# ruc98/Distributed-Data-Parallel-ML-Training

Hardware: AMD Instinct MI355X
Metric: images/sec (whole node) VGG-11 CIFAR-10 (higher is better)
Workload: dtype bf16; 1 GPU; model=vgg11, global_batch=256, per_gpu_batch=256, parallelism=dp1, hipgraph=True, buckets=1, grad_comm=fp32, comm=inline, optimizer=SGD(lr=0.1, momentum=0.9, wd=1e-4) fused

## Files before the change

distributed-data-parallel-ml-training_amd/csrc/bind.cpp:

```cpp
#include <hip/hip_runtime.h>
#include <pybind11/pybind11.h>
#include <pybind11/stl.h>

#include <stdexcept>
#include <string>
#include <tuple>
#include <vector>

#include "runtime/comm.h"

namespace py = pybind11;
using ddp_amd::BucketSpec;
using ddp_amd::RcclComm;
using ddp_amd::Reducer;

#include "kernels/api.h"

template <typename T>
static T* P(uintptr_t v) { return reinterpret_cast<T*>(v); }
static hipStream_t S(uintptr_t v) { return reinterpret_cast<hipStream_t>(v); }
static void check(int rc, const char* what) {
  if (rc != 0) {
    std::string msg = std::string(what) + " failed: ";
    msg += (rc > 0) ? hipGetErrorString((hipError_t)rc) : "invalid arguments";
// ... 469 lines not shown
      return;
    }
    check(ddp_softmax_ce(P<void>(logits), bf16, P<long long>(labels), B, J, P<float>(loss_sum),
                         P<int>(correct), P<void>(dlogits), dlogits_bf16, S(st)), "softmax_ce");
  }, py::arg("logits"), py::arg("bf16"), py::arg("labels"), py::arg("B"), py::arg("J"),
     py::arg("loss_sum"), py::arg("correct"), py::arg("dlogits"), py::arg("dlogits_bf16"),
     py::arg("stream"), py::arg("soft") = py::none());

  m.def("sgd", [](uintptr_t p, uintptr_t g, uintptr_t buf, size_t n, float lr, float momentum,
                  float wd, float grad_scale, int nesterov, uintptr_t st, uintptr_t sched) {
    check(ddp_sgd(P<float>(p), P<float>(g), P<float>(buf), n, lr, momentum, wd, grad_scale,
                  nesterov, P<const ddp_amd::LrSched>(sched), S(st)), "sgd");
  }, py::arg("p"), py::arg("g"), py::arg("buf"), py::arg("n"), py::arg("lr"), py::arg("momentum"),
     py::arg("wd"), py::arg("grad_scale"), py::arg("nesterov"), py::arg("stream"),
     py::arg("sched") = 0);
  m.def("conv_options", [](int stages) { ddp_conv_options(stages); }, py::arg("stages") = 2);
  m.def("conv_tune_set", [](int mode, int M, int N, int K, int tile, int splits, int stages) {
    ddp_conv_tune_set(mode, M, N, K, tile, splits, stages);
  }, py::arg("mode"), py::arg("M"), py::arg("N"), py::arg("K"), py::arg("tile"),
     py::arg("splits"), py::arg("stages") = 0);
  m.def("conv_tune_clear", []() { ddp_conv_tune_clear(); });
  m.def("conv_wgrad_pm_set", [](int on) { ddp_conv_wgrad_pm_set(on); });
  m.def("conv_rows_pm_set", [](int on) { ddp_conv_rows_pm_set(on); });
  m.def("bn_fold_bwd_mb", [](int mb) { ddp_bn_fold_bwd_mb(mb); });
  m.def("bn_fold_grid", [](int blocks) { ddp_bn_fold_grid(blocks); });
  m.def("conv_pair_tune_set", [](int M, int N, int K, int hw, int tile, int sd, int sw) {
    ddp_conv_pair_tune_set(M, N, K, hw, tile, sd, sw);
  });
  m.def("conv_force_tile", [](int t, int stages) { ddp_conv_force_tile(t, stages); },
        py::arg("tile_plus_one"), py::arg("stages") = 0);
#ifdef DDP_CONV_STAMPS
  m.def("conv_stamps_set", [](uintptr_t buf, int cap) { ddp_conv_stamps_set(P<void>(buf), cap); });
#endif
  m.def("pack_conv_weights", [](const std::vector<PackTuple>& descs, uintptr_t st) {
    auto d = pack_descs(descs);
    check(ddp_pack_conv_weights(d.data(), (int)d.size(), S(st)), "pack_conv_weights");
  });
  m.def("sgd_pack", [](uintptr_t items, int n_items, uintptr_t descs, uintptr_t p, uintptr_t g,
                       uintptr_t buf, float lr, float momentum, float wd, float grad_scale,
                       int nesterov, uintptr_t st, int zero_grad, uintptr_t counter, int delta,
                       uintptr_t skip, uintptr_t shadow, uintptr_t slot, uintptr_t done,
                       uintptr_t signal, uintptr_t sched, int sched_advance, uintptr_t lars_side,
                       uintptr_t lars_tensors, uintptr_t lars_partial, uintptr_t lars_trust,
                       float lars_eta, float lars_eps, uintptr_t clip_partial, int clip_chunks,
                       float clip_max_norm, float clip_eps, int clip_flags,
                       uintptr_t clip_stats, uintptr_t ema, float ema_one_minus_decay) {
// ... 247 lines not shown
```

distributed-data-parallel-ml-training_amd/csrc/kernels/api.h:

```cpp
#pragma once
#include <hip/hip_runtime.h>
#include <stddef.h>
#include <stdint.h>

namespace ddp_amd {

#ifdef DDP_AMD_DETERMINISTIC
constexpr int kStatRep = 4096;
constexpr bool kDeterministic = true;
#else
constexpr int kStatRep = 16;
constexpr bool kDeterministic = false;
#endif

struct ConvGeom {
  int N, H, W, C;
  int K;
  int R, S, stride, pad;
  int P, Q;
  int Creal;
  int wkrsc;
};

struct BnArgs {
// ... 277 lines not shown
void ddp_conv_epi_stage_set(int on);
int ddp_bn_pool3_fwd(const ddp_amd::BnArgs* a, unsigned char* idx, hipStream_t st);
int ddp_bn_pool3_bwd(const ddp_amd::BnArgs* a, const unsigned char* idx, hipStream_t st);
void ddp_conv_pair_mode(int mode, int items);
void ddp_sgd_fuse_register(float* dw, const ddp_amd::SgdFuse* f, int clear);
void ddp_sgd_fuse_begin();
int ddp_l0_ok(const ddp_amd::ConvGeom* g);
int ddp_l0_fwd(const ddp_amd::ConvGeom* g, const ddp_amd::L0Io* io, hipStream_t st);
int ddp_l0_bwd(const ddp_amd::ConvGeom* g, const ddp_amd::L0Io* io, hipStream_t st);
int ddp_conv_wgrad_final(const ddp_amd::ConvGeom* g, const void* dy, const void* x, float* dw,
                         float* ws, size_t ws_elems, int splits, hipStream_t st);
int ddp_sgd_fuse_taken(uintptr_t* out, int cap);
int ddp_sgd_fuse_take_final(const float* dw, ddp_amd::SgdFuse* out);
int ddp_sgd_fuse_taken_master(uintptr_t* out, int cap);
void ddp_conv_pair_force(int splits_dg, int splits_wg, int tile);
int ddp_conv_bwd_pair(const ddp_amd::ConvGeom* g, const void* dy, const void* wc, void* dx,
                      const void* x, float* dw, float* ws, size_t ws_elems,
                      const ddp_amd::BnBwdFuse* bn, const ddp_amd::BnBwdApply* ba, int* bn_done,
                      hipStream_t st);
void ddp_conv_tune_set(int mode, int M, int N, int K, int tile, int splits, int stages);
void ddp_conv_pair_tune_set(int M, int N, int K, int hw, int tile, int sd, int sw);
void ddp_conv_wgrad_pm_set(int on);
void ddp_conv_rows_pm_set(int on);
void ddp_bn_fold_bwd_mb(int mb);
void ddp_bn_fold_grid(int blocks);
int ddp_conv_dense2x2_ok(const ddp_amd::ConvGeom* g);
void ddp_conv_dense2x2_set(int on);
void ddp_conv_tune_clear();
void ddp_conv_force_tile(int tile_plus_one, int stages);
#ifdef DDP_CONV_STAMPS
void ddp_conv_stamps_set(void* buf, int cap);
#endif
int ddp_pack_conv_weights(const ddp_amd::PackDesc* descs, int n, hipStream_t st);
int ddp_sgd_pack(const ddp_amd::UpdateLaunch* u, hipStream_t st);
int ddp_grad_sumsq(const void* items, int n_items, const float* g, float grad_scale,
                   float* partial, hipStream_t st);
int ddp_lars_norms(const void* items, int n_items, const float* p, const float* g,
                   float grad_scale, void* partial, hipStream_t st);
int ddp_shard_tail(const void* segs, int n_segs, const float* src, float* dst,
                   const ddp_amd::PackDesc* pack, int n_pack, unsigned* done, unsigned* signal,
                   const unsigned* skip, hipStream_t st);
void ddp_sgd_tile_dims(int RS, int* TK, int* TC);
int ddp_sgd_tile_limit();
int ddp_counter_add(int* c, int delta, ddp_amd::LrSched* sched, int sched_mode, hipStream_t st);
int ddp_synth_generate(unsigned char* images, int* labels, int n, int pix_per_img,
                       unsigned int seed, int classes, hipStream_t st);
// ... 25 lines not shown
```

distributed-data-parallel-ml-training_amd/csrc/kernels/common.h:

```cpp
#pragma once
#include <hip/hip_runtime.h>
#include <stdint.h>
#include <cstdlib>

#include "api.h"

namespace ddp_amd {

typedef __bf16 bf16x8 __attribute__((ext_vector_type(8)));
typedef float f32x4 __attribute__((ext_vector_type(4)));
typedef float f32x16 __attribute__((ext_vector_type(16)));
typedef unsigned short u16x8 __attribute__((ext_vector_type(8)));

constexpr int kWave = 64;

#ifdef DDP_AMD_DEBUG
#define DDP_DEVICE_CHECK(cond)                                                              \
  do {                                                                                      \
    if (!(cond)) {                                                                          \
      printf("[ddp_amd debug] %s:%d check failed: %s (block %d thread %d)\n", __FILE__,     \
             __LINE__, #cond, (int)blockIdx.x, (int)threadIdx.x);                           \
      return;                                                                               \
    }                                                                                       \
  } while (0)
#else
#define DDP_DEVICE_CHECK(cond) \
  do {                        \
  } while (0)
// ... 60 lines not shown
}
__device__ __forceinline__ float dpp_sum16(float v) {
  v += dpp_f<0xB1>(v);
  v += dpp_f<0x4E>(v);
  v += dpp_f<0x141>(v);
  v += dpp_f<0x140>(v);
  return v;
}
__device__ __forceinline__ float lane_f(float v, int l) {
  return __int_as_float(__builtin_amdgcn_readlane(__float_as_int(v), l));
}
__device__ __forceinline__ float wave_sum(float v) {
  v = dpp_sum16(v);
  return (lane_f(v, 0) + lane_f(v, 16)) + (lane_f(v, 32) + lane_f(v, 48));
}
__device__ __forceinline__ float wave_max(float v) {
  v = fmaxf(v, dpp_f<0xB1>(v));
  v = fmaxf(v, dpp_f<0x4E>(v));
  v = fmaxf(v, dpp_f<0x141>(v));
  v = fmaxf(v, dpp_f<0x140>(v));
  return fmaxf(fmaxf(lane_f(v, 0), lane_f(v, 16)), fmaxf(lane_f(v, 32), lane_f(v, 48)));
}

__device__ __forceinline__ int xcd_remap(int orig, int nwg) {
  const int nx = 8;
  if (nwg < nx) return orig;
  const int q = nwg / nx, r = nwg % nx;
  const int xcd = orig % nx, idx = orig / nx;
  return (xcd < r ? xcd * (q + 1) : r * (q + 1) + (xcd - r) * q) + idx;
}

struct FastDiv {
  unsigned mul;
  int sh;
};
__device__ __forceinline__ int fast_div(int x, FastDiv d) {
  return (int)((__umulhi((unsigned)x, d.mul) + (unsigned)x) >> d.sh);
}
inline FastDiv make_fastdiv(int d) {
  FastDiv f;
  int sh = 0;
  while ((1ll << sh) < d) ++sh;
  f.sh = sh;
  f.mul = (unsigned)((((1ull << sh) - (unsigned long long)d) << 32) / (unsigned long long)d + 1);
  return f;
}

#ifdef DDP_CONV_STAMPS
struct ConvStampBuf {
  unsigned* buf;
  int cap;
};
extern ConvStampBuf g_conv_stamps;
__device__ __forceinline__ unsigned long long stamp_now() {
  __builtin_amdgcn_sched_barrier(0);
  const unsigned long long t = __builtin_readcyclecounter();
  __builtin_amdgcn_sched_barrier(0);
  return t;
}
__device__ __forceinline__ void stamp_put(const ConvStampBuf& s, unsigned tag, unsigned long long t0,
                                          unsigned long long t1, unsigned long long t2,
                                          unsigned long long t3) {
  if (!s.buf || threadIdx.x != 0) return;
  const unsigned i = atomicAdd(s.buf, 1u);
  if (i >= (unsigned)s.cap) return;
  unsigned* r = s.buf + 4 + 4 * (size_t)i;
  r[0] = tag;
  r[1] = (unsigned)(t1 - t0);
  r[2] = (unsigned)(t2 - t1);
  r[3] = (unsigned)(t3 - t2);
// ... 15 lines not shown
```

distributed-data-parallel-ml-training_amd/csrc/kernels/conv_igemm.hip:

```cpp
#include "common.h"
#include "api.h"
#include "linear_blocks.h"
#include <algorithm>
#include <map>
#include <set>
#include <cstdlib>

namespace ddp_amd {

enum { MODE_FWD = 0, MODE_DGRAD = 1, MODE_WGRAD = 2 };

typedef short v4i16 __attribute__((ext_vector_type(4)));
typedef short short8_t __attribute__((ext_vector_type(8)));
typedef __attribute__((address_space(3))) v4i16 lds_v4i16;

__global__ __launch_bounds__(256) void zero16_kernel(uint4* __restrict__ p, size_t n16) {
  for (size_t i = blockIdx.x * 256ull + threadIdx.x; i < n16; i += (size_t)gridDim.x * 256)
    p[i] = (uint4){0u, 0u, 0u, 0u};
}

__device__ __forceinline__ void ld8f_conv(const float* p, float* v) {
  const float4 a = reinterpret_cast<const float4*>(p)[0];
  const float4 b = reinterpret_cast<const float4*>(p)[1];
  v[0] = a.x; v[1] = a.y; v[2] = a.z; v[3] = a.w;
  v[4] = b.x; v[5] = b.y; v[6] = b.z; v[7] = b.w;
}
// ... 10 lines not shown
  int Mg, Ng, Kg;
  int splits;
  int ksteps_per_split;
  int phase;
  int pa, pb, Hp, Wp, r0, s0, Rt, St, qa, qb;
  int accumulate;
  int a_bytes, b_bytes;
  FastDiv dPQ, dQ;
  int has_bnf;
  BnBwdFuse bnf;
  const BnFwdFuse* bnfwd;
  int* bnfwd_done;
  const BnBwdApply* bnapply;
  int* bnapply_done;
  int epi_stage;
  int d2x2;
  int d2C, d2K;
  int no_finish;
  const unsigned short* acc_dy;
  const unsigned char* acc_mask;
  SgdFuse sgd;
  int pixmajor;
  FastDiv dTiles, dTilesN, dN, dCdim, dKb, dSdec, dS, dC, dNb, dD2C, dD2K, dSplits;
  int w_dq, w_dp;
#ifdef DDP_CONV_STAMPS
  ConvStampBuf stamps;
#endif
};

__device__ __forceinline__ uint2 acc_old4(const unsigned short* dx, const unsigned short* acc_dy,
                                          const unsigned char* acc_mask, size_t e) {
  if (!acc_mask) return *reinterpret_cast<const uint2*>(dx + e);
  uint2 v = *reinterpret_cast<const uint2*>(acc_dy + e);
  const unsigned mb = (unsigned)acc_mask[e >> 3] >> (e & 4);
  v.x &= ((mb & 1u) ? 0xFFFFu : 0u) | ((mb & 2u) ? 0xFFFF0000u : 0u);
  v.y &= ((mb & 4u) ? 0xFFFFu : 0u) | ((mb & 8u) ? 0xFFFF0000u : 0u);
  return v;
}
__device__ __forceinline__ u16x8 acc_old8(const unsigned short* dx, const unsigned short* acc_dy,
                                          const unsigned char* acc_mask, size_t e) {
  if (!acc_mask) return ld8(dx + e);
  u16x8 v = ld8(acc_dy + e);
  const unsigned mb = acc_mask[e >> 3];
#pragma unroll
  for (int i = 0; i < 8; ++i) v[i] = ((mb >> i) & 1u) ? v[i] : (unsigned short)0;
  return v;
// ... 72 lines not shown

__device__ __forceinline__ void dma_buf(__amdgpu_buffer_rsrc_t rs, int byte_off,
                                        unsigned short* lds_wave_base) {
  __builtin_amdgcn_raw_ptr_buffer_load_lds(rs, (lds_void*)lds_wave_base, 16, byte_off, 0, 0, 0);
}
__device__ __forceinline__ void dma_buf_s(__amdgpu_buffer_rsrc_t rs, int byte_off, int soff,
                                          unsigned short* lds_wave_base) {
  __builtin_amdgcn_raw_ptr_buffer_load_lds(rs, (lds_void*)lds_wave_base, 16, byte_off,
                                           __builtin_amdgcn_readfirstlane(soff), 0, 0);
}

template <int N>
__device__ __forceinline__ void wait_dma_barrier() {
  asm volatile("s_waitcnt vmcnt(%0)\n\ts_barrier" ::"n"(N) : "memory");
}

template <int BM, int BN, int NST>
struct ConvSmem {
  static constexpr int elems = NST * (BM + BN) * 64;
};

template <int MODE, int BM, int BN, int NST, int BNF = 0, bool XSTAT = false, bool SGDM = false>
__device__ __forceinline__ void conv_igemm_body(const ConvArgs& args, unsigned short* smem,
                                                const int bid, const int nblk) {
  constexpr int BK = 64;
  constexpr int WTM = BM / 2, WTN = BN / 2;
  constexpr bool kOldBnf = BNF == 1 || (BNF == 2 && BM == 64 && BN == 64);
  constexpr int TM = WTM / 16, TN = WTN / 16;
  constexpr int CA = BM * BK / 8 / 256;
  constexpr int CB = BN * BK / 8 / 256;
  constexpr int TILE_A = BM * BK, TILE_B = BN * BK;
  constexpr int STAGE = TILE_A + TILE_B;
  static_assert(CA >= 1 && CB >= 1, "tile too small for 256 threads");
  static_assert(NST >= 2 && NST <= 4, "2..4 LDS stages");

  const int tid = threadIdx.x;
  const int lane = tid & 63;
  const int wid = __builtin_amdgcn_readfirstlane(tid >> 6);
  const int wm = wid >> 1, wn = wid & 1;
  DDP_DEVICE_CHECK(blockDim.x == 256 && args.g.C % 8 == 0 && args.g.K % 8 == 0);
  DDP_DEVICE_CHECK(args.splits >= 1 && args.ksteps_per_split >= 1);

  const int tiles_n = (args.Ng + BN - 1) / BN;
  const int tiles_m = (args.Mg + BM - 1) / BM;
  const int tiles = tiles_m * tiles_n;
  const int nitems = tiles * args.splits;
  const int ksteps = (args.Kg + BK - 1) / BK;

  f32x4 acc[TM][TN];
  const ConvGeom& gg = args.g;

  constexpr int NA = (MODE != MODE_WGRAD) ? CA : 1;
  int a_off[CA];
  int a_h0[NA], a_w0[NA];
  int b_off[CB];
  int kr = 0, ks_ = 0, kc = 0;
  KInfo xk;
  int xk_same = 0;
  int wp[CB], wq[CB];
  int w_rr = 0, w_ss = 0, w_lim = 0;
  const bool wsame = MODE == MODE_WGRAD && gg.stride == 1 && gg.P == gg.H && gg.Q == gg.W;
  const int w_dq = args.w_dq;
  const int w_dp = args.w_dp;
  const int w_dm = wsame ? 2 * BK * gg.C : 0;
  const bool pm = MODE == MODE_WGRAD && args.pixmajor;
  const bool pmr = MODE != MODE_WGRAD && args.pixmajor;
  int pmr_pq = 0, pmr_n0 = 0, pmr_row0 = 0, pmr_t = 0;
  int pmr_pp = 0, pmr_qq = 0;
  unsigned pmr_mask = 0;
  int pm_p = 0, pm_q = 0, pm_qlo = 0, pm_qhi = 0, pm_n0 = 0, pm_r = 0, pm_s = 0;
  int row0 = 0, col0 = 0, zsplit = 0, ks_begin = 0, ks_end = 0, cur_tile = 0;
  int d2pos = 0;
  const bool phase = MODE == MODE_DGRAD && args.phase;
  const int Sdec = phase ? args.St : gg.S;
  const int cdim = MODE == MODE_FWD ? gg.C : gg.K;
  const bool fast = MODE != MODE_WGRAD && (cdim % BK) == 0;
  const int lcA = (MODE != MODE_WGRAD) ? ((tid & 7) ^ ((tid >> 4) & 7))
                                       : ((tid % (BM / 8)) ^ mc_swz<BM>(tid / (BM / 8)));
  constexpr bool BKM = MODE != MODE_FWD;
  const int lcB = !BKM ? lcA : ((tid % (BN / 8)) ^ mc_swz<BN>(tid / (BN / 8)));
  const __amdgpu_buffer_rsrc_t rsA = make_rsrc(args.a, args.a_bytes);
  const __amdgpu_buffer_rsrc_t rsB = make_rsrc(args.b, args.b_bytes);

  auto setup = [&](int item) {
    zsplit = fast_div(item, args.dTiles);
    const int tile = xcd_remap(item - zsplit * tiles, tiles);
    cur_tile = tile;
    const int tm = fast_div(tile, args.dTilesN);
    const int tn = tile - tm * tiles_n;
    row0 = tm * BM;
    col0 = tn * BN;
    ks_begin = zsplit * args.ksteps_per_split;
    ks_end = min(ksteps, ks_begin + args.ksteps_per_split);
    if (MODE != MODE_WGRAD) {
      if (pmr) {
        pmr_pq = fast_div(row0, args.dN);
        pmr_n0 = row0 - pmr_pq * gg.N;
        pmr_row0 = row0;
        pmr_pp = fast_div(pmr_pq, args.dQ);
        pmr_qq = pmr_pq - pmr_pp * gg.Q;
        const int img = MODE == MODE_FWD ? gg.H * gg.W * gg.C : gg.P * gg.Q * gg.K;
#pragma unroll
        for (int i = 0; i < CA; ++i) a_off[i] = 2 * (((tid >> 3) + 32 * i) * img + lcA * 8);
      } else {
#pragma unroll
        for (int i = 0; i < CA; ++i) {
          const RowInfo ri = row_info<MODE>(args, row0 + (tid >> 3) + 32 * i);
          a_h0[i] = ri.h0;
          a_w0[i] = ri.w0;
          const int e = (MODE == MODE_FWD) ? ri.base + (ri.h0 * gg.W + ri.w0) * gg.C
                                           : ri.base + (ri.h0 * gg.Q + ri.w0) * gg.K;
          a_off[i] = 2 * (e + (fast ? lcA * 8 : 0));
// ... 716 lines not shown
    }
  }
  if (red) {
    __syncthreads();
    if (wm == 0 && rl == 0) {
      float* st = (MODE == MODE_FWD ? args.stats : args.bnf.sums) +
                  stat_rep(bid) * 2 * args.Ng;
#pragma unroll
      for (int j = 0; j < TN; ++j) {
        const int col = col0 + wn * WTN + j * 16 + cq;
        if (col >= args.Ng) continue;
        const float* slot = reinterpret_cast<const float*>(smem) + (((wn * TN + j) * 4 + (lane >> 4)) * 8);
#pragma unroll
        for (int t = 0; t < 4; ++t) {
          atomicAdd(st + col + t, stat_val(stat_s[j][t] + slot[t], bid));
          atomicAdd(st + args.Ng + col + t, stat_val(stat_ss[j][t] + slot[4 + t], bid));
        }
      }
    }
  }
  };

  constexpr int DMA = CA + CB;
  for (int item = bid; item < nitems; item += nblk) {
#ifdef DDP_CONV_STAMPS
    const unsigned long long st0 = stamp_now();
#endif
    setup(item);
#ifdef DDP_CONV_STAMPS
    const unsigned long long st1 = stamp_now();
#endif
#pragma unroll
    for (int i = 0; i < TM; ++i)
#pragma unroll
      for (int j = 0; j < TN; ++j) acc[i][j] = (f32x4){0.f, 0.f, 0.f, 0.f};
    const int kb = ks_begin, ke = ks_end;
#pragma unroll
    for (int s = 0; s < NST - 1; ++s)
      if (kb + s < ke) issue(kb + s, s);
    int stage = 0;
    for (int ks = kb; ks < ke; ++ks) {
      const int ahead = ke - 1 - ks;
      if (NST >= 4 && ahead >= 2) wait_dma_barrier<(NST >= 4 ? 2 : 0) * DMA>();
      else if (NST >= 3 && ahead >= 1) wait_dma_barrier<(NST >= 3 ? 1 : 0) * DMA>();
      else wait_dma_barrier<0>();
      bf16x8 fa0[TM], fb0[TN], fa1[TM], fb1[TN];
      load_frags(stage, 0, fa0, fb0);
      if (ks + NST - 1 < ke) issue(ks + NST - 1, stage == 0 ? NST - 1 : stage - 1);
      load_frags(stage, 32, fa1, fb1);
      mma(fa0, fb0);
      mma(fa1, fb1);
// ... 19 lines not shown
#define DDP_CONV_WAVES_PER_EU 2
#endif
template <int MODE, int BM, int BN, int NST, int BNF = 0, bool XSTAT = false>
__global__ __launch_bounds__(256) __attribute__((amdgpu_waves_per_eu(DDP_CONV_WAVES_PER_EU)))
void conv_igemm_kernel(ConvArgs args) {
  extern __shared__ __attribute__((aligned(16))) unsigned short smem[];
  conv_igemm_body<MODE, BM, BN, NST, BNF, XSTAT>(args, smem, blockIdx.x, gridDim.x);
}

template <int MODE, int BM, int BN, int NST>
__global__ __launch_bounds__(256) __attribute__((amdgpu_waves_per_eu(2)))
void conv_igemm_bnf2_kernel(ConvArgs args) {
  extern __shared__ __attribute__((aligned(16))) unsigned short smem[];
  conv_igemm_body<MODE, BM, BN, NST, 2>(args, smem, blockIdx.x, gridDim.x);
}

template <int BM, int BN, int NST, int BNF, bool SGDM = false>
__global__ __launch_bounds__(256) void conv_bwd_pair_kernel(ConvArgs dg, ConvArgs wg, int n_dg) {
  __shared__ __attribute__((aligned(16))) unsigned short smem[ConvSmem<BM, BN, NST>::elems];
  if ((int)blockIdx.x < n_dg)
    conv_igemm_body<MODE_DGRAD, BM, BN, NST, BNF>(dg, smem, blockIdx.x, n_dg);
  else
    conv_igemm_body<MODE_WGRAD, BM, BN, NST, 0, false, SGDM>(wg, smem, blockIdx.x - n_dg,
                                                           gridDim.x - n_dg);
}
struct RowMap {
  int stride, Hp, Wp, H, W, pa, pb;
};

__device__ __forceinline__ size_t map_row(const RowMap& m, int row) {
  if (m.stride == 0) return row;
  const int hw = m.Hp * m.Wp;
  const int n = row / hw, rem = row - n * hw;
  const int i = rem / m.Wp, j = rem - i * m.Wp;
  return ((size_t)n * m.H + m.pa + m.stride * i) * m.W + m.pb + m.stride * j;
}

constexpr int kSlabBatch = 8;
__device__ __forceinline__ void sum_slabs8(const float* p, size_t slab, int z0, int z1, float* v) {
  for (int zb = z0; zb < z1; zb += kSlabBatch) {
    float4 a[kSlabBatch], b[kSlabBatch];
#pragma unroll
    for (int u = 0; u < kSlabBatch; ++u) {
      if (zb + u < z1) {
        const float4* src = reinterpret_cast<const float4*>(p + (size_t)(zb + u) * slab);
        a[u] = src[0];
        b[u] = src[1];
// ... 662 lines not shown
  const double eff = (BM == 128 && BN == 128) ? 1.0 : ((BM == 64 && BN == 64) ? 0.55 : 0.8);
  const int resident = (BM == 128 && BN == 128) ? 2 : ((BM == 64 && BN == 64) ? 4 : 3);
  const double blocks = (double)tiles * splits;
  const double fill = std::min(1.0, blocks / (256.0 * resident));
  const double work = (double)tiles * BM * BN * ksteps * 64.0;
  const double t_mfma = work / (eff * fill) / 1.0e15 * 2.0;
  double t_split = 0.0;
  if (splits > 1) t_split = 8.0 * splits * (double)slab / 4.0e12 + 3.0e-6;
  return t_mfma + t_split;
}

static int stages_for(int BM, int BN) {
  if (g_stages <= 2) return 2;
  if (BM == 128 && BN == 128) return g_stages >= 4 ? 4 : 2;
  if (BM == 64 && BN == 64) return g_stages >= 4 ? 4 : 3;
  return 3;
}

static int fwd_stat_grid() {
  constexpr int g = 2048;
  return (kDeterministic ? std::min(g, kStatRep) : g) / 8 * 8;
}

template <int MODE, int BM, int BN, int NST, int BNF>
static void launch_gemm_t(const ConvArgs& a, int items, hipStream_t st) {
  constexpr int kStageBytes = (BM + BN) * 64 * 2;
  constexpr int kTileBytes = BM * BN * 2;
  const int stages = std::max(1, std::min(NST, a.ksteps_per_split));
  size_t lds = (size_t)stages * kStageBytes;
  if (a.epi_stage && lds < (size_t)kTileBytes) lds = kTileBytes;
  int grid = items;
  if (MODE == MODE_FWD && a.stats && a.splits <= 1 && a.epi_stage && !(BM == 64 && BN == 64) &&
      fwd_stat_grid() > 0 && items > fwd_stat_grid())
    grid = fwd_stat_grid();
  void (*kern)(ConvArgs);
  if constexpr (BNF == 2 && MODE == MODE_DGRAD) kern = conv_igemm_bnf2_kernel<MODE, BM, BN, NST>;
  else if constexpr (MODE == MODE_FWD && BNF == 0 && !(BM == 64 && BN == 64))
    kern = grid < items ? conv_igemm_kernel<MODE, BM, BN, NST, 0, true>
                        : conv_igemm_kernel<MODE, BM, BN, NST, 0, false>;
  else kern = conv_igemm_kernel<MODE, BM, BN, NST, BNF>;
  static bool attr[2] = {false, false};
  if (!attr[grid < items]) {
    (void)hipFuncSetAttribute(reinterpret_cast<const void*>(kern),
                              hipFuncAttributeMaxDynamicSharedMemorySize,
                              std::max(NST * kStageBytes, kTileBytes));
    attr[grid < items] = true;
  }
  hipLaunchKernelGGL(kern, dim3(grid), dim3(256), lds, st, a);
}

template <int MODE, int BM, int BN, int NST>
static void launch_gemm(const ConvArgs& a, int items, hipStream_t st) {
  if constexpr (MODE == MODE_DGRAD) {
    if (a.has_bnf && a.splits <= 1)
      return a.bnf.pool ? launch_gemm_t<MODE, BM, BN, NST, 1>(a, items, st)
                        : launch_gemm_t<MODE, BM, BN, NST, 2>(a, items, st);
  }
// ... 42 lines not shown
  {
    const ConvGeom& g = a.g;
    const int cdim = MODE == MODE_FWD ? g.C : g.K;
    const bool wsame = MODE == MODE_WGRAD && g.stride == 1 && g.P == g.H && g.Q == g.W;
    a.dTiles = make_fastdiv(std::max(1, tiles));
    a.dTilesN = make_fastdiv(std::max(1, (a.Ng + BN - 1) / BN));
    a.dN = make_fastdiv(std::max(1, g.N));
    a.dCdim = make_fastdiv(std::max(1, cdim));
    a.dKb = make_fastdiv(std::max(1, cdim / BK));
    a.dSdec = make_fastdiv(std::max(1, MODE == MODE_DGRAD && a.phase ? a.St : g.S));
    a.dS = make_fastdiv(std::max(1, g.S));
    a.dC = make_fastdiv(std::max(1, g.C));
    a.dNb = make_fastdiv(std::max(1, g.N / BK));
    a.dD2C = make_fastdiv(std::max(1, a.d2C));
    a.dD2K = make_fastdiv(std::max(1, a.d2K));
    a.dSplits = make_fastdiv(splits);
    a.w_dq = wsame ? BK % g.Q : 0;
    a.w_dp = wsame ? (BK / g.Q) % g.P : 0;
  }
#ifdef DDP_CONV_STAMPS
  a.stamps = g_conv_stamps;
#endif
  return tiles * splits;
}

static bool needs_finish(int mode, const ConvArgs& a) {
  (void)mode;
  return a.splits > 1;
}

static int finish_rows_per_thread(int Mg, int rows_per_block) {
  return (Mg + rows_per_block - 1) / rows_per_block <= 128 ? 1 : 2;
}

static void dg_finish_grid(const ConvArgs& a, int* bx_out, int* chunks_out) {
  const int G = a.Ng / 8;
  const int Gb = G < 256 ? G : 256;
  const int chunks = (G + Gb - 1) / Gb;
  const int rows_per_block = std::max(1, 256 / Gb);
  const int rpt = finish_rows_per_thread(a.Mg, rows_per_block);
  int bx = (a.Mg + rows_per_block * rpt - 1) / (rows_per_block * rpt);
  *bx_out = std::max(1, std::min(bx, 2048 / chunks + 1));
  *chunks_out = chunks;
}

static FinishArgs finish_args(int mode, const ConvArgs& a) {
// ... 119 lines not shown
    hipLaunchKernelGGL(wgrad_finish_krsc_kernel, dim3(w.gx, w.gy), dim3(256), 0, st, a.ws,
                       a.splits, a.g.K, a.g.R * a.g.S, a.g.C, a.g.Creal, a.dw, w.sgd);
  } else if (MODE == MODE_WGRAD) {
    const int groups = (a.splits + kWgFinishGroup - 1) / kWgFinishGroup;
    const size_t lds = sizeof(float) * a.g.R * a.g.S * a.g.C;
    hipLaunchKernelGGL(wgrad_finish_kernel, dim3(a.g.K, groups), dim3(256), lds, st, a.ws,
                       a.splits, a.g.K, a.g.R, a.g.S, a.g.C, a.g.Creal, a.dw);
  } else {
    if (MODE == MODE_FWD && a.bnfwd && launch_finish_bnfwd(a, st)) return;
    if (MODE == MODE_DGRAD && a.has_bnf && a.bnapply && launch_finish_bnbwd(a, st, nullptr)) return;
    int bx, chunks;
    dg_finish_grid(a, &bx, &chunks);
    const FinishArgs fa = finish_args(MODE, a);
    if (MODE == MODE_DGRAD && a.has_bnf)
      hipLaunchKernelGGL(splitk_finish_kernel<true>, dim3(bx, chunks), dim3(256), 0, st, fa);
    else
      hipLaunchKernelGGL(splitk_finish_kernel<false>, dim3(bx, chunks), dim3(256), 0, st, fa);
  }
}

template <int MODE, int BM, int BN>
static void launch_cfg(ConvArgs& a, int splits, hipStream_t st, int nst_req = 0) {
  const int items = prepare_cfg<MODE, BM, BN>(a, splits);
  constexpr int kStageBytes = (BM + BN) * 64 * 2;
  constexpr int kMaxStages = kStageBytes * 4 <= 163840 ? 4 : (kStageBytes * 3 <= 163840 ? 3 : 2);
  int nst = nst_req >= 2 && nst_req <= 4 ? nst_req : stages_for(BM, BN);
  nst = std::min(nst, kMaxStages);
  if constexpr (kMaxStages >= 4) {
    if (nst == 4) { launch_gemm<MODE, BM, BN, 4>(a, items, st); goto launched; }
  }
  if constexpr (kMaxStages >= 3) {
    if (nst == 3) { launch_gemm<MODE, BM, BN, 3>(a, items, st); goto launched; }
  }
  launch_gemm<MODE, BM, BN, 2>(a, items, st);
launched:
  if (!a.no_finish) launch_finish<MODE>(a, st);
}

struct TuneKey {
  int mode, M, N, K;
  int hw = 0;
  bool operator<(const TuneKey& o) const {
    if (mode != o.mode) return mode < o.mode;
    if (M != o.M) return M < o.M;
    if (N != o.N) return N < o.N;
    if (K != o.K) return K < o.K;
// ... 423 lines not shown
}

constexpr int kPairTiles = 6;
template <int BM, int BN, int NST, bool BNF1, bool SGDM>
static void pair_kernel_launch(const ConvArgs& d, const ConvArgs& w, int itd, int itw,
                               hipStream_t st) {
  hipLaunchKernelGGL((conv_bwd_pair_kernel<BM, BN, NST, BNF1 ? 1 : 0, SGDM>), dim3(itd + itw),
                     dim3(256), 0, st, d, w, itd);
}
template <int BM, int BN, int NST>
static void pair_launch_t(ConvArgs& d, ConvArgs& w, int sd, int sw, float* ws, size_t ws_elems,
                          int* itd_out, int* itw_out, bool* ok_out, const float* dw,
                          bool launch, hipStream_t st) {
  const int itd = prepare_cfg<MODE_DGRAD, BM, BN>(d, std::max(1, sd));
  size_t dneed = needs_finish(MODE_DGRAD, d) ? (size_t)d.splits * d.Mg * d.Ng : 0;
  dneed = (dneed + 63) / 64 * 64;
  w.ws = ws + dneed;
  const int itw = prepare_cfg<MODE_WGRAD, BM, BN>(w, std::max(1, sw));
  const size_t wneed = needs_finish(MODE_WGRAD, w) ? (size_t)w.splits * w.Mg * w.Ng : 0;
  *itd_out = itd;
  *itw_out = itw;
  *ok_out = dneed + wneed <= ws_elems;
  if (!launch || !*ok_out) return;
  if (!needs_finish(MODE_WGRAD, w) && w.g.wkrsc && w.g.Creal == w.g.C) w.sgd = sgd_fuse_master(dw);
  const bool bnf1 = d.has_bnf && d.splits <= 1;
  const bool sgdm = w.sgd.p != nullptr;
  if (bnf1 && sgdm) pair_kernel_launch<BM, BN, NST, true, true>(d, w, itd, itw, st);
  else if (bnf1) pair_kernel_launch<BM, BN, NST, true, false>(d, w, itd, itw, st);
  else if (sgdm) pair_kernel_launch<BM, BN, NST, false, true>(d, w, itd, itw, st);
  else pair_kernel_launch<BM, BN, NST, false, false>(d, w, itd, itw, st);
}

extern "C" int ddp_conv_bwd_pair(const ConvGeom* g, const void* dy, const void* wc, void* dx,
                                 const void* x, float* dw, float* ws, size_t ws_elems,
                                 const BnBwdFuse* bn, const BnBwdApply* ba, int* bn_done,
                                 hipStream_t st) {
  if (bn_done) *bn_done = 0;
  if (!bn) ba = nullptr;
  auto separate = [&]() -> int {
    const BnBwdFuse* bsep = bn && bn->code ? nullptr : bn;
    const int r = conv_dgrad_impl(g, dy, wc, dx, ws, ws_elems, 0, 0, bsep, bsep ? ba : nullptr,
                                  bn_done, st);
    if (r) return r;
    g_sgd_allow = true;
    const int rw = ddp_conv_wgrad(g, dy, x, dw, ws, ws_elems, 0, st);
    g_sgd_allow = false;
// ... 165 lines not shown
```

distributed-data-parallel-ml-training_amd/csrc/kernels/conv_tr.hip:

```cpp
#include "common.h"
#include "api.h"

#include <algorithm>
#include <cstdlib>
#include <map>
#include <tuple>

namespace ddp_amd {
namespace tr {

typedef __attribute__((address_space(3))) void lds_void;

constexpr unsigned kOOB = 0x80000000u;

__device__ __forceinline__ __amdgpu_buffer_rsrc_t make_rsrc(const void* base, int bytes) {
  return __builtin_amdgcn_make_buffer_rsrc(const_cast<void*>(base), (short)0, bytes, 0x00020000);
}

__device__ __forceinline__ void dma(__amdgpu_buffer_rsrc_t rs, unsigned byte_off, unsigned short* lds) {
  __builtin_amdgcn_raw_ptr_buffer_load_lds(rs, (lds_void*)lds, 16, (int)byte_off, 0, 0, 0);
}

template <int N>
__device__ __forceinline__ void wait_dma_barrier() {
// ... 24 lines not shown
  int N, H, W, C, K;
  const unsigned short* x;
  const unsigned short* wc;
  const float* bias;
  unsigned short* z;
  float* stats;
  float* ws;
  int splits, cbps;
  int imgs, rows, bands;
  int imgp, plane, zslot;
  int x_bytes, w_bytes;
  int tiles_m, tiles_n;
  int abuf_elems;
  const unsigned short* zin;
  const float* in_stats;
  const float* in_gamma;
  const float* in_beta;
  float in_eps;
  int in_relu;
  float* in_coef;
  unsigned short* y_out;
  int z_bytes;
  FastDiv dTiles, dTilesN, dBands, dPw, dW, dPerImg;
#ifdef DDP_CONV_STAMPS
  ConvStampBuf stamps;
#endif
};

template <int BM, int BN, int NST, int NL, int IN>
#ifndef DDP_TR_WAVES_PER_EU
#define DDP_TR_WAVES_PER_EU 1
#endif
__global__ __launch_bounds__(256) __attribute__((amdgpu_waves_per_eu(DDP_TR_WAVES_PER_EU)))
void conv_tr_fwd_kernel(Args a) {
  constexpr int WTM = BM / 2, WTN = BN / 2, TM = WTM / 16, TN = WTN / 16;
  constexpr int CB = BN * 64 / 8 / 256;
  constexpr int BTILE = BN * 64;
  static_assert(CB >= 1 && TM >= 1 && TN >= 1, "tile");
  static_assert(NST >= 3 && NST <= 9, "the next patch is issued at tap 0: at most one in the window");
  extern __shared__ __attribute__((aligned(16))) unsigned short smem[];
  const int aelems = a.abuf_elems;
  unsigned short* abuf = smem;
  unsigned short* bring = smem + 2 * aelems;
  float* cf = reinterpret_cast<float*>(bring + NST * BTILE);
  constexpr int NP = IN == 2 ? 4 : 1;
  constexpr bool BNIN = IN == 1 || IN == 2;

  const int tid = threadIdx.x, lane = tid & 63;
  const int wid = __builtin_amdgcn_readfirstlane(tid >> 6);
  const int wm = wid >> 1, wn = wid & 1;
  const int W = a.W, H = a.H, C = a.C, K = a.K;
  const int M = a.N * H * W;
#ifdef DDP_CONV_STAMPS
  const unsigned long long st0 = stamp_now();
#endif
  const int ncb = C / 64;

  const int tiles = a.tiles_m * a.tiles_n;
  const int item = blockIdx.x;
  const int sp = fast_div(item, a.dTiles);
  const int tile = xcd_remap(item - sp * tiles, tiles);
  const int tm = fast_div(tile, a.dTilesN);
  const int tn = tile - tm * a.tiles_n;
  const int row0 = tm * BM, col0 = tn * BN;
  const int cb0 = sp * a.cbps, cb1 = min(ncb, cb0 + a.cbps);
  const int nsteps = (cb1 - cb0) * 9;
  const int tband = fast_div(tm, a.dBands);
  const int n0 = tband * a.imgs;
  const int h0 = (tm - tband * a.bands) * a.rows;

  const __amdgpu_buffer_rsrc_t rsA = IN ? make_rsrc(a.zin, a.z_bytes) : make_rsrc(a.x, a.x_bytes);
  if (BNIN) {
    const int Hz = IN == 2 ? 2 * H : H, Wz = IN == 2 ? 2 * W : W;
    const float Mz = (float)a.N * Hz * Wz;
    for (int c = tid; c < C; c += 256) {
      float s1 = 0.f, s2 = 0.f;
#pragma unroll
      for (int r = 0; r < kStatRep; ++r) {
        s1 += a.in_stats[r * 2 * C + c];
        s2 += a.in_stats[r * 2 * C + C + c];
      }
      const float mu = s1 / Mz;
      const float var = fmaxf(s2 / Mz - mu * mu, 0.f);
      const float is = rsqrtf(var + a.in_eps);
      const float sc = a.in_gamma[c] * is, sh = a.in_beta[c] - mu * sc;
      cf[c] = sc;
// ... 511 lines not shown
  Args a{};
  a.N = N; a.H = H; a.W = W; a.C = C; a.K = K;
  a.x = (const unsigned short*)x;
  a.wc = (const unsigned short*)wc;
  a.bias = bias;
  a.z = (unsigned short*)z;
  a.stats = stats;
  a.ws = ws;
  a.splits = pl.splits;
  a.cbps = pl.cbps;
  a.imgs = geo.imgs; a.rows = geo.rows; a.bands = geo.bands;
  a.imgp = geo.imgp; a.plane = geo.plane; a.zslot = geo.zslot;
  a.x_bytes = (int)(2 * M * C);
  a.w_bytes = (int)(2 * (size_t)K * 9 * C);
  a.abuf_elems = geo.abuf;
  a.tiles_m = (int)(M / c.bm);
  a.tiles_n = K / c.bn;
  a.dTiles = make_fastdiv(std::max(1, a.tiles_m * a.tiles_n));
  a.dTilesN = make_fastdiv(std::max(1, a.tiles_n));
  a.dBands = make_fastdiv(std::max(1, geo.bands));
  a.dPw = make_fastdiv((geo.rows + 2) * W);
  a.dW = make_fastdiv(W);
  a.dPerImg = make_fastdiv(geo.rows * W);
  if (in) {
    a.zin = (const unsigned short*)in->z;
    a.in_stats = in->stats;
    a.in_gamma = in->gamma;
    a.in_beta = in->beta;
    a.in_eps = in->eps;
    a.in_relu = in->relu;
    a.in_coef = in->coef;
    a.y_out = (unsigned short*)in->y;
    a.z_bytes = (int)(2 * M * C * (in->pool ? 4 : 1));
  }
#ifdef DDP_CONV_STAMPS
  a.stamps = g_conv_stamps;
#endif
  const int items = a.tiles_m * a.tiles_n * pl.splits;
  if (!launch_stages(c, in_mode, a, geo.nl, items, st)) return 0;
  int e = (int)hipGetLastError();
  if (e) return 2 + e;
  if (pl.splits > 1) {
    e = ddp_conv_fwd_finish(g, ws, pl.splits, bias, z, stats, bn, bn_done, st);
    if (e) return 2 + e;
  }
  return 1;
// ... 16 lines not shown
```

Baseline: 380,500 images/s.

## Choose conv work-item ordering per XCD via host-side L2 traffic model

```diff
diff --git a/distributed-data-parallel-ml-training_amd/csrc/bind.cpp b/distributed-data-parallel-ml-training_amd/csrc/bind.cpp
--- a/distributed-data-parallel-ml-training_amd/csrc/bind.cpp
+++ b/distributed-data-parallel-ml-training_amd/csrc/bind.cpp
@@ -515,6 +515,7 @@
   m.def("conv_tune_clear", []() { ddp_conv_tune_clear(); });
   m.def("conv_wgrad_pm_set", [](int on) { ddp_conv_wgrad_pm_set(on); });
   m.def("conv_rows_pm_set", [](int on) { ddp_conv_rows_pm_set(on); });
+  m.def("conv_item_order", [](int order) { ddp_conv_item_order(order); });
   m.def("bn_fold_bwd_mb", [](int mb) { ddp_bn_fold_bwd_mb(mb); });
   m.def("bn_fold_grid", [](int blocks) { ddp_bn_fold_grid(blocks); });
   m.def("conv_pair_tune_set", [](int M, int N, int K, int hw, int tile, int sd, int sw) {
diff --git a/distributed-data-parallel-ml-training_amd/csrc/kernels/api.h b/distributed-data-parallel-ml-training_amd/csrc/kernels/api.h
--- a/distributed-data-parallel-ml-training_amd/csrc/kernels/api.h
+++ b/distributed-data-parallel-ml-training_amd/csrc/kernels/api.h
@@ -323,6 +323,8 @@
 void ddp_conv_pair_tune_set(int M, int N, int K, int hw, int tile, int sd, int sw);
 void ddp_conv_wgrad_pm_set(int on);
 void ddp_conv_rows_pm_set(int on);
+void ddp_conv_item_order(int order);
+int ddp_conv_item_order_get();
 void ddp_bn_fold_bwd_mb(int mb);
 void ddp_bn_fold_grid(int blocks);
 int ddp_conv_dense2x2_ok(const ddp_amd::ConvGeom* g);
diff --git a/distributed-data-parallel-ml-training_amd/csrc/kernels/common.h b/distributed-data-parallel-ml-training_amd/csrc/kernels/common.h
--- a/distributed-data-parallel-ml-training_amd/csrc/kernels/common.h
+++ b/distributed-data-parallel-ml-training_amd/csrc/kernels/common.h
@@ -4,6 +4,7 @@
 #include <cstdlib>
 
 #include "api.h"
+#include "conv_item_map.h"
 
 namespace ddp_amd {
 
@@ -110,30 +111,6 @@
   return fmaxf(fmaxf(lane_f(v, 0), lane_f(v, 16)), fmaxf(lane_f(v, 32), lane_f(v, 48)));
 }
 
-__device__ __forceinline__ int xcd_remap(int orig, int nwg) {
-  const int nx = 8;
-  if (nwg < nx) return orig;
-  const int q = nwg / nx, r = nwg % nx;
-  const int xcd = orig % nx, idx = orig / nx;
-  return (xcd < r ? xcd * (q + 1) : r * (q + 1) + (xcd - r) * q) + idx;
-}
-
-struct FastDiv {
-  unsigned mul;
-  int sh;
-};
-__device__ __forceinline__ int fast_div(int x, FastDiv d) {
-  return (int)((__umulhi((unsigned)x, d.mul) + (unsigned)x) >> d.sh);
-}
-inline FastDiv make_fastdiv(int d) {
-  FastDiv f;
-  int sh = 0;
-  while ((1ll << sh) < d) ++sh;
-  f.sh = sh;
-  f.mul = (unsigned)((((1ull << sh) - (unsigned long long)d) << 32) / (unsigned long long)d + 1);
-  return f;
-}
-
 #ifdef DDP_CONV_STAMPS
 struct ConvStampBuf {
   unsigned* buf;
diff --git a/distributed-data-parallel-ml-training_amd/csrc/kernels/conv_igemm.hip b/distributed-data-parallel-ml-training_amd/csrc/kernels/conv_igemm.hip
--- a/distributed-data-parallel-ml-training_amd/csrc/kernels/conv_igemm.hip
+++ b/distributed-data-parallel-ml-training_amd/csrc/kernels/conv_igemm.hip
@@ -2,6 +2,7 @@
 #include "api.h"
 #include "linear_blocks.h"
 #include <algorithm>
+#include <array>
 #include <map>
 #include <set>
 #include <cstdlib>
@@ -58,6 +59,7 @@
   SgdFuse sgd;
   int pixmajor;
   FastDiv dTiles, dTilesN, dN, dCdim, dKb, dSdec, dS, dC, dNb, dD2C, dD2K, dSplits;
+  int item_order;
   int w_dq, w_dp;
 #ifdef DDP_CONV_STAMPS
   ConvStampBuf stamps;
@@ -176,7 +178,8 @@
 
 template <int MODE, int BM, int BN, int NST, int BNF = 0, bool XSTAT = false, bool SGDM = false>
 __device__ __forceinline__ void conv_igemm_body(const ConvArgs& args, unsigned short* smem,
-                                                const int bid, const int nblk) {
+                                                const int bid, const int nblk,
+                                                const int first = 0) {
   constexpr int BK = 64;
   constexpr int WTM = BM / 2, WTN = BN / 2;
   constexpr bool kOldBnf = BNF == 1 || (BNF == 2 && BM == 64 && BN == 64);
@@ -200,7 +203,6 @@
   const int tiles = tiles_m * tiles_n;
   const int nitems = tiles * args.splits;
   const int ksteps = (args.Kg + BK - 1) / BK;
-
   f32x4 acc[TM][TN];
   const ConvGeom& gg = args.g;
 
@@ -236,12 +238,14 @@
   const __amdgpu_buffer_rsrc_t rsA = make_rsrc(args.a, args.a_bytes);
   const __amdgpu_buffer_rsrc_t rsB = make_rsrc(args.b, args.b_bytes);
 
-  auto setup = [&](int item) {
-    zsplit = fast_div(item, args.dTiles);
-    const int tile = xcd_remap(item - zsplit * tiles, tiles);
-    cur_tile = tile;
-    const int tm = fast_div(tile, args.dTilesN);
-    const int tn = tile - tm * tiles_n;
+  auto setup = [&](int k) {
+    const int order = args.item_order;
+    const item_map::Walk walk = item_map::walk_begin(order, first + bid, first, nblk, nitems);
+    const item_map::Dims dims{tiles_m, tiles_n, args.splits, args.dTiles, args.dTilesN};
+    const int lin = walk.base + k * walk.stride;
+    int tm, tn;
+    item_map::decode(order, lin, dims, &zsplit, &tm, &tn);
+    cur_tile = tm * tiles_n + tn;
     row0 = tm * BM;
     col0 = tn * BN;
     ks_begin = zsplit * args.ksteps_per_split;
@@ -1004,11 +1008,11 @@
   };
 
   constexpr int DMA = CA + CB;
-  for (int item = bid; item < nitems; item += nblk) {
+  for (int item = bid, k = 0; item < nitems; item += nblk, ++k) {
 #ifdef DDP_CONV_STAMPS
     const unsigned long long st0 = stamp_now();
 #endif
-    setup(item);
+    setup(k);
 #ifdef DDP_CONV_STAMPS
     const unsigned long long st1 = stamp_now();
 #endif
@@ -1074,7 +1078,7 @@
     conv_igemm_body<MODE_DGRAD, BM, BN, NST, BNF>(dg, smem, blockIdx.x, n_dg);
   else
     conv_igemm_body<MODE_WGRAD, BM, BN, NST, 0, false, SGDM>(wg, smem, blockIdx.x - n_dg,
-                                                           gridDim.x - n_dg);
+                                                           gridDim.x - n_dg, n_dg);
 }
 struct RowMap {
   int stride, Hp, Wp, H, W, pa, pb;
@@ -1783,6 +1787,14 @@
   return (kDeterministic ? std::min(g, kStatRep) : g) / 8 * 8;
 }
 
+template <int MODE, int BM, int BN>
+static int gemm_grid(const ConvArgs& a, int items) {
+  if (MODE == MODE_FWD && a.stats && a.splits <= 1 && a.epi_stage && !(BM == 64 && BN == 64) &&
+      fwd_stat_grid() > 0 && items > fwd_stat_grid())
+    return fwd_stat_grid();
+  return items;
+}
+
 template <int MODE, int BM, int BN, int NST, int BNF>
 static void launch_gemm_t(const ConvArgs& a, int items, hipStream_t st) {
   constexpr int kStageBytes = (BM + BN) * 64 * 2;
@@ -1790,10 +1802,7 @@
   const int stages = std::max(1, std::min(NST, a.ksteps_per_split));
   size_t lds = (size_t)stages * kStageBytes;
   if (a.epi_stage && lds < (size_t)kTileBytes) lds = kTileBytes;
-  int grid = items;
-  if (MODE == MODE_FWD && a.stats && a.splits <= 1 && a.epi_stage && !(BM == 64 && BN == 64) &&
-      fwd_stat_grid() > 0 && items > fwd_stat_grid())
-    grid = fwd_stat_grid();
+  const int grid = gemm_grid<MODE, BM, BN>(a, items);
   void (*kern)(ConvArgs);
   if constexpr (BNF == 2 && MODE == MODE_DGRAD) kern = conv_igemm_bnf2_kernel<MODE, BM, BN, NST>;
   else if constexpr (MODE == MODE_FWD && BNF == 0 && !(BM == 64 && BN == 64))
@@ -1882,6 +1891,36 @@
   a.stamps = g_conv_stamps;
 #endif
   return tiles * splits;
+}
+
+static int g_item_order = -1;
+extern "C" void ddp_conv_item_order(int order) {
+  g_item_order = order >= 0 && order < item_map::kNumOrders ? order : -1;
+}
+extern "C" int ddp_conv_item_order_get() { return g_item_order; }
+template <int MODE, int BM, int BN>
+static void choose_item_order(ConvArgs& a, int first, int nblk) {
+  const ConvGeom& g = a.g;
+  item_map::ModelProblem p{};
+  p.mode = MODE;
+  p.N = g.N; p.H = g.H; p.W = g.W; p.C = g.C; p.K = g.K; p.R = g.R; p.S = g.S; p.pad = g.pad;
+  p.Mg = a.Mg; p.Ng = a.Ng; p.Kg = a.Kg;
+  p.BM = BM; p.BN = BN;
+  p.splits = a.splits;
+  p.ksteps_per_split = a.ksteps_per_split;
+  p.pixmajor = a.pixmajor;
+  p.first = first;
+  p.nblk = nblk;
+  int order = g_item_order;
+  if (order < 0 || !item_map::order_ok(p, order)) {
+    static std::map<std::array<int, 18>, int> cache;
+    const std::array<int, 18> key{MODE, g.N, g.H, g.W, g.C, g.K, g.R * 64 + g.S, g.pad, a.Mg, a.Ng,
+                                  a.Kg, BM, BN, a.splits, a.ksteps_per_split, a.pixmajor, first, nblk};
+    auto it = cache.find(key);
+    if (it == cache.end()) it = cache.emplace(key, item_map::model_choose(p)).first;
+    order = it->second;
+  }
+  a.item_order = order;
 }
 
 static bool needs_finish(int mode, const ConvArgs& a) {
@@ -2047,6 +2086,7 @@
 template <int MODE, int BM, int BN>
 static void launch_cfg(ConvArgs& a, int splits, hipStream_t st, int nst_req = 0) {
   const int items = prepare_cfg<MODE, BM, BN>(a, splits);
+  choose_item_order<MODE, BM, BN>(a, 0, gemm_grid<MODE, BM, BN>(a, items));
   constexpr int kStageBytes = (BM + BN) * 64 * 2;
   constexpr int kMaxStages = kStageBytes * 4 <= 163840 ? 4 : (kStageBytes * 3 <= 163840 ? 3 : 2);
   int nst = nst_req >= 2 && nst_req <= 4 ? nst_req : stages_for(BM, BN);
@@ -2516,6 +2556,8 @@
   *itw_out = itw;
   *ok_out = dneed + wneed <= ws_elems;
   if (!launch || !*ok_out) return;
+  choose_item_order<MODE_DGRAD, BM, BN>(d, 0, itd);
+  choose_item_order<MODE_WGRAD, BM, BN>(w, itd, itw);
   if (!needs_finish(MODE_WGRAD, w) && w.g.wkrsc && w.g.Creal == w.g.C) w.sgd = sgd_fuse_master(dw);
   const bool bnf1 = d.has_bnf && d.splits <= 1;
   const bool sgdm = w.sgd.p != nullptr;
diff --git a/distributed-data-parallel-ml-training_amd/csrc/kernels/conv_item_map.h b/distributed-data-parallel-ml-training_amd/csrc/kernels/conv_item_map.h
--- /dev/null
+++ b/distributed-data-parallel-ml-training_amd/csrc/kernels/conv_item_map.h
@@ -0,0 +1,232 @@
+#pragma once
+#if defined(__HIPCC__)
+#define DDP_IM_HD __host__ __device__ __forceinline__
+#else
+#define DDP_IM_HD inline
+#endif
+
+namespace ddp_amd {
+
+struct FastDiv {
+  unsigned mul;
+  int sh;
+};
+DDP_IM_HD int fast_div(int x, FastDiv d) {
+  const unsigned hi = (unsigned)(((unsigned long long)(unsigned)x * d.mul) >> 32);
+  return (int)((hi + (unsigned)x) >> d.sh);
+}
+inline FastDiv make_fastdiv(int d) {
+  FastDiv f;
+  int sh = 0;
+  while ((1ll << sh) < d) ++sh;
+  f.sh = sh;
+  f.mul = (unsigned)((((1ull << sh) - (unsigned long long)d) << 32) / (unsigned long long)d + 1);
+  return f;
+}
+
+DDP_IM_HD int xcd_remap(int orig, int nwg) {
+  const int nx = 8;
+  if (nwg < nx) return orig;
+  const int q = nwg / nx, r = nwg % nx;
+  const int xcd = orig % nx, idx = orig / nx;
+  return (xcd < r ? xcd * (q + 1) : r * (q + 1) + (xcd - r) * q) + idx;
+}
+
+namespace item_map {
+
+enum Order { kLegacy = 0, kSplitMajor = 1, kNumOrders = 2 };
+
+struct Dims {
+  int tiles_m, tiles_n, splits;
+  FastDiv dTiles, dTilesN;
+};
+inline Dims make_dims(int tiles_m, int tiles_n, int splits) {
+  Dims d;
+  d.tiles_m = tiles_m;
+  d.tiles_n = tiles_n;
+  d.splits = splits;
+  d.dTiles = make_fastdiv(tiles_m * tiles_n > 0 ? tiles_m * tiles_n : 1);
+  d.dTilesN = make_fastdiv(tiles_n > 0 ? tiles_n : 1);
+  return d;
+}
+
+struct Walk {
+  int base, stride;
+};
+
+DDP_IM_HD int below_class(int x, int c) {
+  const int r = x & 7;
+  return (x >> 3) * c + (r < c ? r : c);
+}
+DDP_IM_HD int in_class(int x, int c) { return (x + 7 - c) >> 3; }
+
+DDP_IM_HD Walk walk_begin(int order, int block, int first, int nblk, int items) {
+  Walk w;
+  const int j = block - first;
+  if (order == kLegacy) {
+    w.base = j;
+    w.stride = nblk;
+    return w;
+  }
+  const int o = first & 7, c = block & 7, jp = j + o;
+  const int omin = o < c ? o : c, own = c < o ? 1 : 0;
+  int rounds = 0, rem = items;
+  if (nblk < items) {
+    rounds = items / nblk;
+    rem = items - rounds * nblk;
+  }
+  w.stride = in_class(o + nblk, c) - own;
+  w.base = rounds * (below_class(o + nblk, c) - omin) + (below_class(o + rem, c) - omin) +
+           (jp >> 3) - own;
+  return w;
+}
+
+DDP_IM_HD void decode(int order, int lin, const Dims& d, int* z, int* tm, int* tn) {
+  const int tiles = d.tiles_m * d.tiles_n;
+  const int zz = fast_div(lin, d.dTiles);
+  int t = lin - zz * tiles;
+  if (order == kLegacy) t = xcd_remap(t, tiles);
+  const int m = fast_div(t, d.dTilesN);
+  *z = zz;
+  *tm = m;
+  *tn = t - m * d.tiles_n;
+}
+
+}
+}
+
+#include <algorithm>
+#include <cstdint>
+#include <vector>
+
+namespace ddp_amd {
+namespace item_map {
+
+struct ModelProblem {
+  int mode;
+  int N, H, W, C, K, R, S, pad;
+  int Mg, Ng, Kg;
+  int BM, BN;
+  int splits, ksteps_per_split;
+  int pixmajor;
+  int first, nblk;
+};
+
+inline int model_tiles_m(const ModelProblem& p) { return (p.Mg + p.BM - 1) / p.BM; }
+inline int model_tiles_n(const ModelProblem& p) { return (p.Ng + p.BN - 1) / p.BN; }
+inline int model_nib(const ModelProblem& p) {
+  return p.pixmajor && p.mode != 2 && p.BM > 0 && p.N >= p.BM ? p.N / p.BM : 1;
+}
+inline bool order_ok(const ModelProblem&, int order) { return order >= 0 && order < kNumOrders; }
+
+inline void model_item_slices(const ModelProblem& p, int z, int tm, int tn,
+                              std::vector<std::pair<uint64_t, uint32_t>>* out) {
+  const uint64_t kA = 1ull << 62, kB = 2ull << 62;
+  const uint32_t bytesA = (uint32_t)p.BM * 64 * 2, bytesB = (uint32_t)p.BN * 64 * 2;
+  auto key = [](uint64_t tag, uint64_t a, uint64_t b, uint64_t c) {
+    return tag | (a << 40) | (b << 20) | c;
+  };
+  if (p.mode == 3) {
+    const int ncb = p.C / 64;
+    for (int cb = z * p.ksteps_per_split; cb < std::min(ncb, (z + 1) * p.ksteps_per_split); ++cb) {
+      out->push_back({key(kA, tm, 0, cb), bytesA});
+      out->push_back({key(kB, tn, 0, cb), bytesB * 9});
+    }
+    return;
+  }
+  const int ksteps = (p.Kg + 63) / 64;
+  if (p.mode != 2) {
+    const int cdim = p.mode == 0 ? p.C : p.K;
+    const int kb = std::max(1, cdim / 64);
+    if (p.pixmajor) {
+      const int nib = model_nib(p), pq = tm / nib, ib = tm - pq * nib;
+      const int pp = pq / p.W, qq = pq - pp * p.W;
+      int taps[32], nt = 0;
+      for (int r = 0; r < p.R; ++r)
+        for (int s = 0; s < p.S; ++s) {
+          const int h = p.mode == 0 ? pp + r - p.pad : pp - r + p.pad;
+          const int w = p.mode == 0 ? qq + s - p.pad : qq - s + p.pad;
+          if (h >= 0 && h < p.H && w >= 0 && w < p.W && nt < 32) taps[nt++] = r * p.S + s;
+        }
+      const int V = nt * kb, per = (V + p.splits - 1) / p.splits;
+      const int b = std::min(V, z * per), e = std::min(V, b + per);
+      for (int ks = b; ks < e; ++ks) {
+        const int t = taps[ks / kb], cb = ks % kb, r = t / p.S, s = t - r * p.S;
+        const int h = p.mode == 0 ? pp + r - p.pad : pp - r + p.pad;
+        const int w = p.mode == 0 ? qq + s - p.pad : qq - s + p.pad;
+        out->push_back({key(kA, ib, h * p.W + w, cb), bytesA});
+        out->push_back({key(kB, tn, 0, t * kb + cb), bytesB});
+      }
+      return;
+    }
+    const int b = z * p.ksteps_per_split, e = std::min(ksteps, b + p.ksteps_per_split);
+    for (int ks = b; ks < e; ++ks) {
+      out->push_back({key(kA, tm, 0, cdim % 64 == 0 ? ks % kb : ks), bytesA});
+      out->push_back({key(kB, tn, 0, ks), bytesB});
+    }
+    return;
+  }
+  const int col0 = tn * p.BN;
+  const int cblk = p.BN < p.C ? (col0 % p.C) / p.BN : 0;
+  if (p.pixmajor) {
+    const int t = col0 / p.C, r = t / p.S, s = t - r * p.S, nb = p.N / 64;
+    const int p_lo = std::max(0, p.pad - r), p_hi = std::min(p.H, p.H + p.pad - r);
+    const int q_lo = std::max(0, p.pad - s), q_hi = std::min(p.W, p.W + p.pad - s);
+    const int nq = std::max(0, q_hi - q_lo), V = std::max(0, p_hi - p_lo) * nq * nb;
+    const int per = (V + p.splits - 1) / p.splits;
+    const int b = std::min(V, z * per), e = std::min(V, b + per);
+    for (int ks = b; ks < e; ++ks) {
+      const int jv = ks / nb, n0 = ks - jv * nb, pp = p_lo + jv / nq, qq = q_lo + jv % nq;
+      out->push_back({key(kA, tm, pp * p.W + qq, n0), bytesA});
+      out->push_back({key(kB, cblk, (pp + r - p.pad) * p.W + (qq + s - p.pad), n0), bytesB});
+    }
+    return;
+  }
+  const int b = z * p.ksteps_per_split, e = std::min(ksteps, b + p.ksteps_per_split);
+  for (int ks = b; ks < e; ++ks) {
+    out->push_back({key(kA, tm, 0, ks), bytesA});
+    out->push_back({key(kB, cblk, 0, ks), bytesB});
+  }
+}
+
+inline double model_bytes(const ModelProblem& p, int order) {
+  const int tiles_m = model_tiles_m(p), tiles_n = model_tiles_n(p);
+  const int items = tiles_m * tiles_n * p.splits;
+  const Dims d = make_dims(tiles_m, tiles_n, p.splits);
+  std::vector<std::pair<uint64_t, uint32_t>> cls[8];
+  for (int blk = p.first; blk < p.first + p.nblk; ++blk) {
+    const Walk w = walk_begin(order, blk, p.first, p.nblk, items);
+    for (int k = 0; (blk - p.first) + (long long)k * p.nblk < items; ++k) {
+      int z, tm, tn;
+      decode(order, w.base + k * w.stride, d, &z, &tm, &tn);
+      model_item_slices(p, z, tm, tn, &cls[blk & 7]);
+    }
+  }
+  double total = 0.0;
+  for (auto& v : cls) {
+    std::sort(v.begin(), v.end());
+    v.erase(std::unique(v.begin(), v.end()), v.end());
+    for (const auto& s : v) total += s.second;
+  }
+  return total;
+}
+
+inline int model_choose(const ModelProblem& p, double* bytes_out = nullptr,
+                        double* per_order = nullptr) {
+  int best = kLegacy;
+  double bb = 0.0;
+  for (int o = 0; o < kNumOrders; ++o) {
+    const bool ok = order_ok(p, o);
+    const double b = ok ? model_bytes(p, o) : -1.0;
+    if (per_order) per_order[o] = b;
+    if (ok && (o == kLegacy || b < bb)) {
+      bb = b;
+      best = o;
+    }
+  }
+  if (bytes_out) *bytes_out = bb;
+  return best;
+}
+
+}
+}
diff --git a/distributed-data-parallel-ml-training_amd/csrc/kernels/conv_tr.hip b/distributed-data-parallel-ml-training_amd/csrc/kernels/conv_tr.hip
--- a/distributed-data-parallel-ml-training_amd/csrc/kernels/conv_tr.hip
+++ b/distributed-data-parallel-ml-training_amd/csrc/kernels/conv_tr.hip
@@ -70,6 +70,7 @@
   unsigned short* y_out;
   int z_bytes;
   FastDiv dTiles, dTilesN, dBands, dPw, dW, dPerImg;
+  int item_order;
 #ifdef DDP_CONV_STAMPS
   ConvStampBuf stamps;
 #endif
@@ -105,11 +106,11 @@
   const int ncb = C / 64;
 
   const int tiles = a.tiles_m * a.tiles_n;
-  const int item = blockIdx.x;
-  const int sp = fast_div(item, a.dTiles);
-  const int tile = xcd_remap(item - sp * tiles, tiles);
-  const int tm = fast_div(tile, a.dTilesN);
-  const int tn = tile - tm * a.tiles_n;
+  const item_map::Walk walk =
+      item_map::walk_begin(a.item_order, blockIdx.x, 0, gridDim.x, tiles * a.splits);
+  const item_map::Dims dims{a.tiles_m, a.tiles_n, a.splits, a.dTiles, a.dTilesN};
+  int sp, tm, tn;
+  item_map::decode(a.item_order, walk.base, dims, &sp, &tm, &tn);
   const int row0 = tm * BM, col0 = tn * BN;
   const int cb0 = sp * a.cbps, cb1 = min(ncb, cb0 + a.cbps);
   const int nsteps = (cb1 - cb0) * 9;
@@ -667,6 +668,26 @@
   a.dPw = make_fastdiv((geo.rows + 2) * W);
   a.dW = make_fastdiv(W);
   a.dPerImg = make_fastdiv(geo.rows * W);
+  {
+    item_map::ModelProblem p{};
+    p.mode = 3;
+    p.N = N; p.H = H; p.W = W; p.C = C; p.K = K; p.R = 3; p.S = 3; p.pad = 1;
+    p.Mg = (int)M; p.Ng = K; p.Kg = C;
+    p.BM = c.bm; p.BN = c.bn;
+    p.splits = pl.splits;
+    p.ksteps_per_split = pl.cbps;
+    p.first = 0;
+    p.nblk = a.tiles_m * a.tiles_n * pl.splits;
+    int order = ddp_conv_item_order_get();
+    if (order < 0 || !item_map::order_ok(p, order)) {
+      static std::map<std::tuple<int, int, int, int, int, int, int>, int> cache;
+      const auto key = std::make_tuple((int)M, K, C, H, c.bm, c.bn, pl.splits);
+      auto it = cache.find(key);
+      if (it == cache.end()) it = cache.emplace(key, item_map::model_choose(p)).first;
+      order = it->second;
+    }
+    a.item_order = order;
+  }
   if (in) {
     a.zin = (const unsigned short*)in->z;
     a.in_stats = in->stats;
```

Measured after the change: 380,600 images/s, median of 2. Within noise of the previous version (+0.0%).
